# zhangyi-3/UCDIR

Measured on AMD Instinct MI355X. Metric: restored images/sec at 50-step p_sample_loop, 256x256 SID, higher is better.
Workload: dtype bf16

## Files before the change

### ucdir_amd/csrc/conv_ws.hip.h

```cpp
#pragma once
#include <type_traits>
#include "akgm_ws.hip.h"

#ifndef CW_DEPTH
#define CW_DEPTH 1
#endif

struct CvWs {
    static constexpr int PITCH = AkWs::PITCH, HALO = AkWs::HALO, QSTEP = AkWs::QSTEP;
    static constexpr int OFF_TCS = 2 * HALO;
    static constexpr int OFF_SCAL = OFF_TCS + 9 * 64 * 4;
    static constexpr int LDS = OFF_SCAL + 128;
    static constexpr int A_ELEMS = 2 * 36 * 2 * 32 * 8;
};

__global__ __launch_bounds__(HC_THREADS, 2) void conv_ws_kernel(const GemmP p) {
    extern __shared__ __attribute__((aligned(16))) unsigned char smem[];
    float* const tcs = reinterpret_cast<float*>(smem + CvWs::OFF_TCS);
    float* const scal = reinterpret_cast<float*>(smem + CvWs::OFF_SCAL);
    const int tid = threadIdx.x, lane = tid & 63, l31 = lane & 31, hh = lane >> 5;
    const int wave = __builtin_amdgcn_readfirstlane(tid >> 6);
    const int rw = wave & 1, pw = wave >> 1;
    const int prow = l31 >> 4, pcol = (l31 & 15) ^ (prow << 3);
    int lid;
    {
        const int nblk = gridDim.x, bid = blockIdx.x;
        const int q = nblk >> 3, r = nblk & 7, xcd = bid & 7;
        lid = (xcd < r ? xcd * (q + 1) : r * (q + 1) + (xcd - r) * q) + (bid >> 3);
    }
#ifdef UCDIR_TIMING
    const bool dbg_on = p.dbg && (lid == (int)gridDim.x / 2 + 3) && (lane == 0) && (wave == 1 || wave == 5);
    unsigned long long* const dbgp = p.dbg + (wave == 5 ? 256 : 0);
    int dbg_n = 0;
#define CW_STAMP() do { if (dbg_on && dbg_n < 250) dbgp[dbg_n++] = __builtin_amdgcn_s_memtime(); } while (0)
#else
#define CW_STAMP() do {} while (0)
#endif
    CW_STAMP();
    const int tps = p.tiles_x * p.tiles_y;
    const int T = p.nbatch * tps;
    const int t_beg = (int)((long long)lid * T / (int)gridDim.x), t_end = (int)((long long)(lid + 1) * T / (int)gridDim.x);
    if (t_beg >= t_end) return;

    bf16x8_t af[36];
    {
        const bf16_t* Ab = p.A + ((rw * 36 * 2 + hh) * 32 + l31) * 8;
#pragma unroll
        for (int j = 0; j < 36; ++j) af[j] = *reinterpret_cast<const bf16x8_t*>(Ab + j * (2 * 32 * 8));
    }
#pragma unroll
    for (int j = 0; j < 36; ++j) asm volatile("" : "+v"(af[j]));

    int hrel[3], hrel_x = -1;
#pragma unroll
    for (int c3 = 0; c3 < 3; ++c3) {
        const int col = c3 * 8 + (lane >> 3), hp = wave * CvWs::PITCH + col;
        hrel[c3] = col < 18 ? (wave * p.Wp + col) * 64 + (((lane & 7) ^ ((hp >> 1) & 7)) << 3) : -1;
    }
    const int xr = 16 + (wave - 2) / 3, xc3 = (wave - 2) % 3;
    if (wave >= 2) {
        const int col = xc3 * 8 + (lane >> 3), hp = xr * CvWs::PITCH + col;
        hrel_x = col < 18 ? (xr * p.Wp + col) * 64 + (((lane & 7) ^ ((hp >> 1) & 7)) << 3) : -1;
    }
    unsigned ba[3][4];
    {
        const int hp0 = (4 * pw + prow) * CvWs::PITCH + pcol;
#pragma unroll
        for (int kx = 0; kx < 3; ++kx) {
            const int sxh = (((hp0 + kx) >> 1) & 7) ^ hh;
#pragma unroll
            for (int k2 = 0; k2 < 4; ++k2) ba[kx][k2] = ((hp0 + kx) << 7) + (((2 * k2) ^ sxh) << 4);
        }
    }
    const unsigned tc_lane = CvWs::OFF_TCS + (32 * rw + 16 * hh) * 4;
    const unsigned rel_out = (unsigned)(((4 * pw + prow + 1) * p.Wp + pcol + 1) * 64 + 32 * rw + 16 * hh) * 2;

    int b, ty, tx;
    {
        b = t_beg / tps;
        const int r = t_beg - b * tps;
        ty = r / p.tiles_x; tx = r - ty * p.tiles_x;
    }
    auto issue_tile = [&](int nb, int nty, int ntx, int buf) {
        const bf16_t* hb = p.B0 + (long long)nb * p.b0_bstride + (long long)(nty * 16 * p.Wp + ntx * 16) * 64;
        unsigned char* hd = smem + buf * CvWs::HALO;
#pragma unroll
        for (int c3 = 0; c3 < 3; ++c3)
            if (hrel[c3] >= 0) {
                stage16(hb + hrel[c3], hd + (3 * wave + c3) * 1024, lane);
                stage16(hb + (long long)8 * p.Wp * 64 + hrel[c3], hd + (3 * (wave + 8) + c3) * 1024, lane);
            }
        if (wave >= 2) { if (hrel_x >= 0) stage16(hb + hrel_x, hd + (3 * xr + xc3) * 1024, lane); }
    };
    issue_tile(b, ty, tx, 0);

    int b_cur = -1;
    float rstd_a = 1.f;
    stat_t S1 = 0, S2 = 0;
    const int act = p.act;

    f32x16_t acc[2];
    bool pend = false;
    int pb = 0, pty = 0, ptx = 0;
    auto epilogue = [&](int eb, int ety, int etx, const bool wait_dma) {
        const bool interior = ety > 0 && etx > 0 && ety + 1 < p.tiles_y && etx + 1 < p.tiles_x;
        unsigned char* outb = reinterpret_cast<unsigned char*>(reinterpret_cast<bf16_t*>(p.out) + (long long)eb * p.out_bstride + (long long)(ety * 16 * p.Wp + etx * 16) * 64);
        float s1 = 0.f, s2 = 0.f;
        uint4 pk[2][2];
#pragma unroll
        for (int tp = 0; tp < 2; ++tp) {
            unsigned tca = tc_lane + 4 * 256;
            if (!interior) {
                const int r = 4 * pw + 2 * tp + prow, c = pcol;
                const int cy = (ety == 0 && r == 0) ? 0 : ((ety + 1 == p.tiles_y && r == 15) ? 2 : 1);
                const int cx = (etx == 0 && c == 0) ? 0 : ((etx + 1 == p.tiles_x && c == 15) ? 2 : 1);
                tca = tc_lane + (cy * 3 + cx) * 256;
            }
            float v[16];
#pragma unroll
            for (int g4 = 0; g4 < 4; ++g4) {
                const f32x4_t c4 = *reinterpret_cast<const f32x4_t*>(smem + tca + 16 * g4);
#pragma unroll
                for (int e = 0; e < 4; ++e) v[4 * g4 + e] = fmaf(acc[tp][4 * g4 + e], rstd_a, c4[e]);
            }
            if (act == 1) {
#pragma unroll
                for (int i = 0; i < 16; ++i) v[i] = silu_fast(v[i]);
            } else if (act == 2) {
#pragma unroll
                for (int i = 0; i < 16; ++i) v[i] = fmaxf(0.2f * v[i], v[i]);
            }
#pragma unroll
            for (int i = 0; i < 16; ++i) { s1 += v[i]; s2 += v[i] * v[i]; }
            pk[tp][0] = pack8_bf16(v); pk[tp][1] = pack8_bf16(v + 8);
        }
        if (wait_dma) { HC_WAIT(0); }
#pragma unroll
        for (int tp = 0; tp < 2; ++tp) {
            unsigned char* op = outb + rel_out + (long long)tp * (2 * p.Wp * 64 * 2);
            *reinterpret_cast<uint4*>(op) = pk[tp][0];
            *reinterpret_cast<uint4*>(op + 16) = pk[tp][1];
        }
        S1 += stat_fx((double)s1); S2 += stat_fx((double)s2);
    };

    auto tile_loop = [&](auto late_tag) {
    constexpr bool late = decltype(late_tag)::value;
#pragma unroll 1
    for (int t = t_beg; t < t_end; ++t) {
        const int buf = (t - t_beg) & 1;
        const bool last = t + 1 == t_end;
        CW_STAMP();
        if (t == t_beg) { HC_WAIT(0); }
        asm volatile("s_barrier" ::: "memory");
        CW_STAMP();
        if (late && pend) { epilogue(pb, pty, ptx, false); pend = false; }
        if (b != b_cur) {
            if (b_cur >= 0 && p.stats_out) {
                const stat_t a = wave_sum_ll(S1), q2 = wave_sum_ll(S2);
                if (lane == 0) stat_add_fx(p.stats_out, b_cur, a, q2);
            }
            S1 = 0; S2 = 0;
            b_cur = b;
            if (wave == 0) {
                float mean = 0.f, rstd = 1.f;
                if (p.fold) {
                    long long v = 0;
                    if (lane < 2 * UCDIR_STAT_SLOTS) v = p.stats0[(long long)b * (2 * UCDIR_STAT_SLOTS) + lane];
#pragma unroll
                    for (int off = 2; off < 2 * UCDIR_STAT_SLOTS; off <<= 1) v += __shfl_xor(v, off);
                    const long long q = __shfl(v, 1);
                    mean_rstd(stat_val(v), stat_val(q), p.inv_count, mean, rstd);
                }
                if (lane == 0) { scal[0] = mean; scal[1] = rstd; }
            }
            __syncthreads();
            const float mean = scal[0], rstd = scal[1];
            for (int i = tid; i < 9 * 64; i += HC_THREADS) {
                const int cls = i >> 6, f = i & 63;
                float v = p.bias ? p.bias[f] : 0.f;
                if (p.fold) v += p.Tb[(long long)cls * p.tab_ld + f] - mean * rstd * p.Tg[(long long)cls * p.tab_ld + f];
                tcs[i] = v;
            }
            rstd_a = __builtin_bit_cast(float, __builtin_amdgcn_readfirstlane(__builtin_bit_cast(int, p.alpha * (p.fold ? rstd : 1.0f))));
            __syncthreads();
        }
        int nb = b, nty = ty, ntx = tx + 1;
        if (ntx == p.tiles_x) { ntx = 0; if (++nty == p.tiles_y) { nty = 0; ++nb; } }
        CW_STAMP();
        if (!last) issue_tile(nb, nty, ntx, buf ^ 1);
        CW_STAMP();

        if (t != t_beg) {
            const int d = buf ? CvWs::HALO : -CvWs::HALO;
#pragma unroll
            for (int kx = 0; kx < 3; ++kx)
#pragma unroll
                for (int k2 = 0; k2 < 4; ++k2) ba[kx][k2] += d;
        }
#pragma unroll
        for (int tp = 0; tp < 2; ++tp)
#pragma unroll
            for (int e = 0; e < 16; ++e) acc[tp][e] = 0.f;
        bf16x8_t bq[3][2];
        auto read_b = [&](auto jc, bf16x8_t (&dst)[2]) {
            constexpr int j = decltype(jc)::value;
            constexpr int tap = j >> 2, c16 = j & 3;
            constexpr int ky = tap / 3, kx = tap - 3 * ky;
            constexpr int k2 = c16 ^ (ky == 1 ? 2 : 0);
            lds_read16_asm<ky * (CvWs::PITCH * 128)>(dst[0], ba[kx][k2]);
            lds_read16_asm<ky * (CvWs::PITCH * 128) + CvWs::QSTEP>(dst[1], ba[kx][k2]);
        };
        __builtin_amdgcn_sched_barrier(0);
        asm volatile("s_waitcnt lgkmcnt(0)" ::: "memory");
        read_b(std::integral_constant<int, 0>{}, bq[0]);
        read_b(std::integral_constant<int, 1>{}, bq[1]);
        __builtin_amdgcn_s_setprio(1);
        static_for<0, 36>([&](auto jc) {
            constexpr int j = decltype(jc)::value;
            if constexpr (j + 2 < 36) read_b(std::integral_constant<int, j + 2>{}, bq[(j + 2) % 3]);
            constexpr int younger = (j + 2 < 36) ? 4 : ((j + 1 < 36) ? 2 : 0);
            lgkm_wait_asm<younger>();
            const f32x16_t zero = {0.f, 0.f, 0.f, 0.f, 0.f, 0.f, 0.f, 0.f, 0.f, 0.f, 0.f, 0.f, 0.f, 0.f, 0.f, 0.f};
            acc[0] = __builtin_amdgcn_mfma_f32_32x32x16_bf16(af[j], bq[j % 3][0], j ? acc[0] : zero, 0, 0, 0);
            acc[1] = __builtin_amdgcn_mfma_f32_32x32x16_bf16(af[j], bq[j % 3][1], j ? acc[1] : zero, 0, 0, 0);
        });
        __builtin_amdgcn_sched_barrier(0);
        __builtin_amdgcn_s_setprio(0);
        CW_STAMP();
        if (late) { HC_WAIT(0); }
        CW_STAMP();
        if (late) { pend = true; pb = b; pty = ty; ptx = tx; } else epilogue(b, ty, tx, true);
        CW_STAMP();
        b = nb; ty = nty; tx = ntx;
    }
    if (late && pend) epilogue(pb, pty, ptx, false);
#ifdef UCDIR_TIMING
    if (dbg_on) dbgp[255] = dbg_n;
#endif
    };
    if (wave >= 4) tile_loop(std::true_type{}); else tile_loop(std::false_type{});
    if (p.stats_out) {
        const stat_t a = wave_sum_ll(S1), q2 = wave_sum_ll(S2);
        if (lane == 0) stat_add_fx(p.stats_out, b_cur, a, q2);
    }
}
```

### ucdir_amd/csrc/conv_ws128.hip.h

```cpp
#pragma once
#include <type_traits>
#include "conv_ws.hip.h"

struct CvWs128 {
    static constexpr int PITCH = 24;
    static constexpr int PLANE = 10 * PITCH * 128;
    static constexpr int HALO = 2 * PLANE;
    static constexpr int QSTEP = 2 * PITCH * 128;
    static constexpr int OFF_A2 = 2 * HALO;
    static constexpr int A2_BYTES = 2 * 8 * 2 * 32 * 16;
    static constexpr int OFF_TCS = OFF_A2 + A2_BYTES;
    static constexpr int OFF_B2 = OFF_TCS + 9 * 64 * 4;
    static constexpr int OFF_SCAL = OFF_B2 + 64 * 4;
    static constexpr int LDS = OFF_SCAL + 128;
    static constexpr int THREADS = 256;
    static constexpr int DEPTH = 3;
};

__global__ __launch_bounds__(CvWs128::THREADS, 1) void conv_ws128_kernel(const GemmP p) {
    using L = CvWs128;
    extern __shared__ __attribute__((aligned(16))) unsigned char smem[];
    float* const tcs = reinterpret_cast<float*>(smem + L::OFF_TCS);
    float* const b2s = reinterpret_cast<float*>(smem + L::OFF_B2);
    float* const scal = reinterpret_cast<float*>(smem + L::OFF_SCAL);
    const int tid = threadIdx.x, lane = tid & 63, l31 = lane & 31, hh = lane >> 5;
    const int wave = __builtin_amdgcn_readfirstlane(tid >> 6);
    const int rw = wave & 1, pw = wave >> 1;
    const int prow = l31 >> 4, pcol = (l31 & 15) ^ (prow << 3);
    int lid;
    {
        const int nblk = gridDim.x, bid = blockIdx.x;
        const int q = nblk >> 3, r = nblk & 7, xcd = bid & 7;
        lid = (xcd < r ? xcd * (q + 1) : r * (q + 1) + (xcd - r) * q) + (bid >> 3);
    }
#ifdef UCDIR_TIMING
    const bool dbg_on = p.dbg && (lid == (int)gridDim.x / 2 + 3) && (lane == 0) && (wave == 1);
    int dbg_n = 0;
#define C8_STAMP() do { if (dbg_on && dbg_n < 250) p.dbg[dbg_n++] = __builtin_amdgcn_s_memtime(); } while (0)
#else
#define C8_STAMP() do {} while (0)
#endif
    C8_STAMP();
    const int tps = p.tiles_x * p.tiles_y;
    const int T = p.nbatch * tps;
    const int t_beg = (int)((long long)lid * T / (int)gridDim.x), t_end = (int)((long long)(lid + 1) * T / (int)gridDim.x);
    if (t_beg >= t_end) return;

    bf16x8_t af[72];
    {
        const bf16_t* Ab = p.A + ((rw * 72 * 2 + hh) * 32 + l31) * 8;
#pragma unroll
        for (int j = 0; j < 72; ++j) af[j] = *reinterpret_cast<const bf16x8_t*>(Ab + j * (2 * 32 * 8));
    }
#pragma unroll
    for (int j = 0; j < 72; ++j) asm volatile("" : "+v"(af[j]));
    for (int i = tid; i < L::A2_BYTES / 16; i += L::THREADS)
        reinterpret_cast<uint4*>(smem + L::OFF_A2)[i] = reinterpret_cast<const uint4*>(p.alt_A)[i];
    if (tid < 64) b2s[tid] = p.bias2 ? p.bias2[tid] : 0.f;
    __syncthreads();

    unsigned hrel[3];
#pragma unroll
    for (int c3 = 0; c3 < 3; ++c3) {
        const int col = c3 * 8 + (lane >> 3), hp = wave * L::PITCH + col;
        hrel[c3] = col < 18 ? (unsigned)((wave * p.Wp + col) * 64 + (((lane & 7) ^ ((hp >> 1) & 7)) << 3)) * 2u : 0xffffffffu;
    }
    unsigned ba[3][4];
    {
        const int hp0 = (4 * pw + prow) * L::PITCH + pcol;
#pragma unroll
        for (int kx = 0; kx < 3; ++kx) {
            const int sxh = (((hp0 + kx) >> 1) & 7) ^ hh;
#pragma unroll
            for (int k2 = 0; k2 < 4; ++k2) ba[kx][k2] = ((hp0 + kx) << 7) + (((2 * k2) ^ sxh) << 4);
        }
    }
    const unsigned tc_lane = L::OFF_TCS + (32 * rw + 16 * hh) * 4;
    const unsigned b2_lane = L::OFF_B2 + (32 * rw + 16 * hh) * 4;
    const unsigned a2_lane = L::OFF_A2 + ((rw * 8 * 2 + hh) * 32 + l31) * 16;
    const unsigned rel_out = (unsigned)(((4 * pw + prow + 1) * p.Wp + pcol + 1) * 64 + 32 * rw + 16 * hh) * 2;

    int b, ty, tx;
    {
        b = t_beg / tps;
        const int r = t_beg - b * tps;
        ty = r / p.tiles_x; tx = r - ty * p.tiles_x;
    }
    auto issue_tile = [&](int nb, int nty, int ntx, int buf) {
        const long long pix0 = (long long)nty * 8 * p.Wp + ntx * 16;
        const unsigned char* h0 = reinterpret_cast<const unsigned char*>(p.B0 + (long long)nb * p.b0_bstride + pix0 * 64);
        const unsigned char* h1 = reinterpret_cast<const unsigned char*>(p.B1 + (long long)nb * p.b1_bstride + pix0 * 64);
        unsigned char* hd = smem + buf * L::HALO;
        const long long r4 = (long long)4 * p.Wp * 64 * 2;
#pragma unroll
        for (int c3 = 0; c3 < 3; ++c3)
            if (hrel[c3] != 0xffffffffu) {
#pragma unroll
                for (int k = 0; k < 3; ++k)
                    if (k < 2 || wave < 2) {
                        stage16(reinterpret_cast<const bf16_t*>(h0 + k * r4 + hrel[c3]), hd + (3 * (wave + 4 * k) + c3) * 1024, lane);
                        stage16(reinterpret_cast<const bf16_t*>(h1 + k * r4 + hrel[c3]), hd + L::PLANE + (3 * (wave + 4 * k) + c3) * 1024, lane);
                    }
            }
    };
    issue_tile(b, ty, tx, 0);

    int b_cur = -1;
    float rstd_a = 1.f;
    stat_t S1 = 0, S2 = 0;
    const int act = p.act;

#pragma unroll 1
    for (int t = t_beg; t < t_end; ++t) {
        const int buf = (t - t_beg) & 1;
        const bool last = t + 1 == t_end;
        C8_STAMP();
        if (t == t_beg) { HC_WAIT(0); }
        asm volatile("s_barrier" ::: "memory");
        C8_STAMP();
        if (b != b_cur) {
            if (b_cur >= 0 && p.stats_out) {
                const stat_t a = wave_sum_ll(S1), q2 = wave_sum_ll(S2);
                if (lane == 0) stat_add_fx(p.stats_out, b_cur, a, q2);
            }
            S1 = 0; S2 = 0;
            b_cur = b;
            if (wave == 0) {
                float mean = 0.f, rstd = 1.f;
                if (p.fold) {
                    long long v = 0;
                    if (lane < 2 * UCDIR_STAT_SLOTS) {
                        v = p.stats0[(long long)b * (2 * UCDIR_STAT_SLOTS) + lane];
                        if (p.stats1) v += p.stats1[(long long)b * (2 * UCDIR_STAT_SLOTS) + lane];
                    }
#pragma unroll
                    for (int off = 2; off < 2 * UCDIR_STAT_SLOTS; off <<= 1) v += __shfl_xor(v, off);
                    const long long q = __shfl(v, 1);
                    mean_rstd(stat_val(v), stat_val(q), p.inv_count, mean, rstd);
                }
                if (lane == 0) { scal[0] = mean; scal[1] = rstd; }
            }
            __syncthreads();
            const float mean = scal[0], rstd = scal[1];
            for (int i = tid; i < 9 * 64; i += L::THREADS) {
                const int cls = i >> 6, f = i & 63;
                float v = p.bias ? p.bias[f] : 0.f;
                if (p.fold) v += p.Tb[(long long)cls * p.tab_ld + f] - mean * rstd * p.Tg[(long long)cls * p.tab_ld + f];
                tcs[i] = v;
            }
            rstd_a = __builtin_bit_cast(float, __builtin_amdgcn_readfirstlane(__builtin_bit_cast(int, p.alpha * (p.fold ? rstd : 1.0f))));
            __syncthreads();
        }
        int nb = b, nty = ty, ntx = tx + 1;
        if (ntx == p.tiles_x) { ntx = 0; if (++nty == p.tiles_y) { nty = 0; ++nb; } }
        C8_STAMP();

        if (t != t_beg) {
            const int d = buf ? L::HALO : -L::HALO;
#pragma unroll
            for (int kx = 0; kx < 3; ++kx)
#pragma unroll
                for (int k2 = 0; k2 < 4; ++k2) ba[kx][k2] += d;
        }

        f32x16_t acc[2];
        {
            bf16x8_t bq[L::DEPTH + 1][2];
            const long long npix0 = (long long)nty * 8 * p.Wp + ntx * 16;
            const unsigned char* h0 = reinterpret_cast<const unsigned char*>(p.B0 + (long long)nb * p.b0_bstride + npix0 * 64);
            const unsigned char* h1 = reinterpret_cast<const unsigned char*>(p.B1 + (long long)nb * p.b1_bstride + npix0 * 64);
            unsigned char* const hd = smem + (buf ^ 1) * L::HALO;
            const long long r4 = (long long)4 * p.Wp * 64 * 2;
            __builtin_amdgcn_sched_barrier(0);
            asm volatile("s_waitcnt lgkmcnt(0)" ::: "memory");
            static_for<0, L::DEPTH>([&](auto jc) {
                constexpr int j = decltype(jc)::value;
                constexpr int tap = j >> 3, c16 = j & 7, ky = tap / 3, kx = tap - 3 * ky;
                constexpr int off = (c16 >> 2) * L::PLANE + ky * (L::PITCH * 128);
                lds_read16_asm<off>(bq[j][0], ba[kx][(c16 & 3) ^ (ky == 1 ? 2 : 0)]);
                lds_read16_asm<off + L::QSTEP>(bq[j][1], ba[kx][(c16 & 3) ^ (ky == 1 ? 2 : 0)]);
            });
            static_for<0, 72>([&](auto jc) {
                constexpr int j = decltype(jc)::value;
                if constexpr (j + L::DEPTH < 72) {
                    constexpr int jn = j + L::DEPTH;
                    constexpr int tap = jn >> 3, c16 = jn & 7, ky = tap / 3, kx = tap - 3 * ky;
                    constexpr int off = (c16 >> 2) * L::PLANE + ky * (L::PITCH * 128);
                    lds_read16_asm<off>(bq[jn % (L::DEPTH + 1)][0], ba[kx][(c16 & 3) ^ (ky == 1 ? 2 : 0)]);
                    lds_read16_asm<off + L::QSTEP>(bq[jn % (L::DEPTH + 1)][1], ba[kx][(c16 & 3) ^ (ky == 1 ? 2 : 0)]);
                }
                if constexpr (j % 4 == 1 && j / 4 < 18) {
                    constexpr int e = j / 4, c3 = e / 6, k = (e % 6) >> 1, pl = e & 1;
                    if (!last && (k < 2 || wave < 2) && hrel[c3] != 0xffffffffu)
                        stage16(reinterpret_cast<const bf16_t*>((pl ? h1 : h0) + k * r4 + hrel[c3]),
                                hd + pl * L::PLANE + (3 * (wave + 4 * k) + c3) * 1024, lane);
                }
                constexpr int ahead = (71 - j) < L::DEPTH ? (71 - j) : L::DEPTH;
                lgkm_wait_asm<2 * ahead>();
                const f32x16_t zero = {0.f, 0.f, 0.f, 0.f, 0.f, 0.f, 0.f, 0.f, 0.f, 0.f, 0.f, 0.f, 0.f, 0.f, 0.f, 0.f};
                acc[0] = __builtin_amdgcn_mfma_f32_32x32x16_bf16(af[j], bq[j % (L::DEPTH + 1)][0], j ? acc[0] : zero, 0, 0, 0);
                acc[1] = __builtin_amdgcn_mfma_f32_32x32x16_bf16(af[j], bq[j % (L::DEPTH + 1)][1], j ? acc[1] : zero, 0, 0, 0);
            });
            __builtin_amdgcn_sched_barrier(0);
        }
        C8_STAMP();
        f32x16_t acc2[2];
        {
            const f32x16_t zero = {0.f, 0.f, 0.f, 0.f, 0.f, 0.f, 0.f, 0.f, 0.f, 0.f, 0.f, 0.f, 0.f, 0.f, 0.f, 0.f};
#pragma unroll
            for (int j = 0; j < 8; ++j) {
                const bf16x8_t a2 = *reinterpret_cast<const bf16x8_t*>(smem + a2_lane + j * 1024);
                const unsigned a0 = ba[1][(j & 3) ^ 2] + (j >> 2) * L::PLANE + L::PITCH * 128;
                const bf16x8_t b0 = *reinterpret_cast<const bf16x8_t*>(smem + a0);
                const bf16x8_t b1 = *reinterpret_cast<const bf16x8_t*>(smem + a0 + L::QSTEP);
                acc2[0] = __builtin_amdgcn_mfma_f32_32x32x16_bf16(a2, b0, j ? acc2[0] : zero, 0, 0, 0);
                acc2[1] = __builtin_amdgcn_mfma_f32_32x32x16_bf16(a2, b1, j ? acc2[1] : zero, 0, 0, 0);
            }
        }

        C8_STAMP();
        const bool interior = ty > 0 && tx > 0 && ty + 1 < p.tiles_y && tx + 1 < p.tiles_x;
        const long long tile_el = (long long)(ty * 8 * p.Wp + tx * 16) * 64;
        unsigned char* outb = reinterpret_cast<unsigned char*>(reinterpret_cast<bf16_t*>(p.out) + (long long)b * p.out_bstride + tile_el);
        unsigned char* out2b = reinterpret_cast<unsigned char*>(p.out2 + (long long)b * p.out2_bstride + tile_el);
        float s1 = 0.f, s2 = 0.f;
        uint4 pk[2][2], pk2[2][2];
#pragma unroll
        for (int tp = 0; tp < 2; ++tp) {
            unsigned tca = tc_lane + 4 * 256;
            if (!interior) {
                const int r = 4 * pw + 2 * tp + prow, c = pcol;
                const int cy = (ty == 0 && r == 0) ? 0 : ((ty + 1 == p.tiles_y && r == 7) ? 2 : 1);
                const int cx = (tx == 0 && c == 0) ? 0 : ((tx + 1 == p.tiles_x && c == 15) ? 2 : 1);
                tca = tc_lane + (cy * 3 + cx) * 256;
            }
            float v[16], w[16];
#pragma unroll
            for (int g4 = 0; g4 < 4; ++g4) {
                const f32x4_t c4 = *reinterpret_cast<const f32x4_t*>(smem + tca + 16 * g4);
                const f32x4_t d4 = *reinterpret_cast<const f32x4_t*>(smem + b2_lane + 16 * g4);
#pragma unroll
                for (int e = 0; e < 4; ++e) {
                    v[4 * g4 + e] = fmaf(acc[tp][4 * g4 + e], rstd_a, c4[e]);
                    w[4 * g4 + e] = acc2[tp][4 * g4 + e] + d4[e];
                }
            }
            if (act == 1) {
#pragma unroll
                for (int i = 0; i < 16; ++i) v[i] = silu_fast(v[i]);
            } else if (act == 2) {
#pragma unroll
                for (int i = 0; i < 16; ++i) v[i] = fmaxf(0.2f * v[i], v[i]);
            }
#pragma unroll
            for (int i = 0; i < 16; ++i) { s1 += v[i]; s2 += v[i] * v[i]; }
            pk[tp][0] = pack8_bf16(v); pk[tp][1] = pack8_bf16(v + 8);
            pk2[tp][0] = pack8_bf16(w); pk2[tp][1] = pack8_bf16(w + 8);
        }
        C8_STAMP();
        HC_WAIT(0);
        C8_STAMP();
#pragma unroll
        for (int tp = 0; tp < 2; ++tp) {
            const long long o = rel_out + (long long)tp * (2 * p.Wp * 64 * 2);
            *reinterpret_cast<uint4*>(outb + o) = pk[tp][0];
            *reinterpret_cast<uint4*>(outb + o + 16) = pk[tp][1];
            *reinterpret_cast<uint4*>(out2b + o) = pk2[tp][0];
            *reinterpret_cast<uint4*>(out2b + o + 16) = pk2[tp][1];
        }
        S1 += stat_fx((double)s1); S2 += stat_fx((double)s2);
        b = nb; ty = nty; tx = ntx;
    }
#ifdef UCDIR_TIMING
    if (dbg_on) p.dbg[255] = dbg_n;
#endif
    if (p.stats_out) {
        const stat_t a = wave_sum_ll(S1), q2 = wave_sum_ll(S2);
        if (lane == 0) stat_add_fx(p.stats_out, b_cur, a, q2);
    }
}
```

### ucdir_amd/csrc/flash_attn2.hip.h

```cpp
#pragma once
#include "cgemm.hip.h"
#include "asmops.hip.h"

typedef __attribute__((ext_vector_type(8))) _Float16 f16x8_t;
typedef __attribute__((ext_vector_type(2))) uint32_t u32x2_t;

struct FlashP {
    const bf16_t* qkv; long long qkv_bstride; int ld;
    const bf16_t* vt; long long vt_bstride; int Npad;
    int N, C, W;
    float scale_log2e;
    const float* bias;
    const bf16_t* res; long long res_bstride;
    bf16_t* out; long long out_bstride;
    stat_t* stats_out;
    int nq;
    unsigned long long* dbg;
};

#ifdef UCDIR_TIMING
#define FA_STAMP() do { if (dbg_on && dbg_n < 250) p.dbg[dbg_n++] = __builtin_amdgcn_s_memtime(); } while (0)
#else
#define FA_STAMP() do {} while (0)
#endif

#define FA_BQ 128
#define FA_BK 64
#define FA_THREADS 512

__host__ __device__ constexpr int fa_lds_bytes(int C) { return FA_BK * C * 2 * 2 + FA_BQ * FA_BK * 2 + 2048; }

template <bool HALF> struct FaVec { typedef bf16x8_t T; };
template <> struct FaVec<true> { typedef f16x8_t T; };
__device__ __forceinline__ f32x4_t fa_mfma16(const bf16x8_t& a, const bf16x8_t& b, f32x4_t c) { return __builtin_amdgcn_mfma_f32_16x16x32_bf16(a, b, c, 0, 0, 0); }
__device__ __forceinline__ f32x4_t fa_mfma16(const f16x8_t& a, const f16x8_t& b, f32x4_t c) { return __builtin_amdgcn_mfma_f32_16x16x32_f16(a, b, c, 0, 0, 0); }
__device__ __forceinline__ f32x16_t fa_mfma32(const bf16x8_t& a, const bf16x8_t& b, f32x16_t c) { return __builtin_amdgcn_mfma_f32_32x32x16_bf16(a, b, c, 0, 0, 0); }
__device__ __forceinline__ f32x16_t fa_mfma32(const f16x8_t& a, const f16x8_t& b, f32x16_t c) { return __builtin_amdgcn_mfma_f32_32x32x16_f16(a, b, c, 0, 0, 0); }
template <bool HALF>
__device__ __forceinline__ uint32_t fa_pack2(float lo, float hi) {
    if constexpr (HALF) {
        typedef __attribute__((ext_vector_type(2))) _Float16 h2;
        h2 v; v[0] = (_Float16)lo; v[1] = (_Float16)hi;
        return __builtin_bit_cast(uint32_t, v);
    } else return pack2_bf16(lo, hi);
}

template <int OFF, typename V>
__device__ __forceinline__ void fa2_read16(V& v, unsigned addr) {
    asm volatile("ds_read_b128 %0, %1 offset:%2" : "=v"(v) : "v"(addr), "n"(OFF));
}

template <int NC, bool HALF>
__global__ __launch_bounds__(FA_THREADS, 2) void flash_attn2_kernel(const FlashP p) {
    extern __shared__ __attribute__((aligned(16))) unsigned char smem[];
    constexpr int C = 128 * NC;
    constexpr int KROW = C * 2;
    constexpr int NKS = C / 32;
    unsigned char* Kl = smem;
    unsigned char* Vl = smem + FA_BK * KROW;
    unsigned char* Pl = Vl + C * (FA_BK * 2);
    float* rowsc = reinterpret_cast<float*>(Pl + FA_BQ * FA_BK * 2);
    float* red = rowsc + 256;

    const int tid = threadIdx.x, lane = tid & 63;
    const int wave = __builtin_amdgcn_readfirstlane(tid >> 6);
    int lid;
    {
        const int nblk = gridDim.x, bid = blockIdx.x;
        const int q = nblk >> 3, r = nblk & 7, xcd = bid & 7;
        lid = (xcd < r ? xcd * (q + 1) : r * (q + 1) + (xcd - r) * q) + (bid >> 3);
    }
    const int b = lid / p.nq, qtile = lid - b * p.nq;
    const int q0 = qtile * FA_BQ;
    const int N = p.N;
    const int ntiles = (N + FA_BK - 1) / FA_BK;
    const bf16_t* qkvb = p.qkv + (long long)b * p.qkv_bstride;
    const bf16_t* vtb = p.vt + (long long)b * p.vt_bstride;

    const unsigned char* kglob = reinterpret_cast<const unsigned char*>(qkvb + C);
    const unsigned char* vglob = reinterpret_cast<const unsigned char*>(vtb);
    const unsigned krow_bytes = (unsigned)p.ld * 2, vrow_bytes = (unsigned)p.Npad * 2;
    constexpr int NPIECE = 2 * NC;
    auto issue_K_piece = [&](int t, int i) {
        constexpr int LPR = KROW / 16;
        int ln = lane;
        asm volatile("" : "+v"(ln));
        const int inst = i * 8 + wave;
        if constexpr (LPR == 64) {
            int kg = t * FA_BK + inst; kg = kg < N ? kg : N - 1;
            const unsigned char* rowp = kglob + (size_t)__builtin_amdgcn_readfirstlane(kg) * krow_bytes;
            dma16_sbase(rowp, (unsigned)((ln ^ (inst & 15)) << 4), (unsigned)__builtin_amdgcn_readfirstlane(inst * 1024));
        } else {
            const int e = inst * 64 + ln, r = e / LPR, j = e - r * LPR;
            int kg = t * FA_BK + r; kg = kg < N ? kg : N - 1;
            const unsigned off = (unsigned)kg * krow_bytes + (unsigned)((j ^ (r & 15)) << 4);
            dma16_sbase(kglob, off, (unsigned)__builtin_amdgcn_readfirstlane(inst * 1024));
        }
    };
    auto issue_K = [&](int t) {
#pragma unroll
        for (int i = 0; i < NPIECE; ++i) issue_K_piece(t, i);
    };
    auto issue_V_piece = [&](int t, int i) {
        int ln = lane;
        asm volatile("" : "+v"(ln));
        const unsigned lc = (unsigned)((ln & 7) ^ (ln >> 4) ^ ((wave & 1) << 2));
        const unsigned off = (unsigned)(ln >> 3) * vrow_bytes + lc * 16;
        const int inst = i * 8 + wave;
        const unsigned char* rowp = vglob + (size_t)(inst * 8) * vrow_bytes + (size_t)t * (FA_BK * 2);
        dma16_sbase(rowp, off, (unsigned)__builtin_amdgcn_readfirstlane(FA_BK * KROW + inst * 1024));
    };

#ifdef UCDIR_TIMING
    const bool dbg_on = p.dbg && (lid == (int)gridDim.x / 2) && (lane == 0) && (wave == 5);
    int dbg_n = 0;
#endif
    FA_STAMP();
    issue_K(0);

    const int x = lane & 15, g = lane >> 4;
    typedef typename FaVec<HALF>::T vec_t;
    vec_t qf[NKS];
    {
        int qg = q0 + 16 * wave + x; qg = qg < N ? qg : N - 1;
        const bf16_t* qp = qkvb + (long long)qg * p.ld + 8 * g;
#pragma unroll
        for (int ks = 0; ks < NKS; ++ks) qf[ks] = *reinterpret_cast<const vec_t*>(qp + 32 * ks);
    }

    const int kbase = x * KROW, kxor = (g ^ x) << 4;
    const int h = lane >> 5, l31 = lane & 31;
    const int qh = wave >> 2, dq = wave & 3;
    const int vbase = l31 * 128, vxor = (h ^ ((l31 >> 1) & 7)) << 4;
    const int pwbase = (16 * wave + x) * 128 + (g & 1) * 8, pwxor = ((g >> 1) ^ ((x >> 1) & 7)) << 4;

    f32x16_t oacc[NC][2];
#pragma unroll
    for (int dt = 0; dt < NC; ++dt)
#pragma unroll
        for (int qt = 0; qt < 2; ++qt)
#pragma unroll
            for (int e = 0; e < 16; ++e) oacc[dt][qt][e] = 0.f;
    float m_run = -1.0e30f, l_run = 0.f;
    const float c1 = p.scale_log2e;
    constexpr int DPW = 32 * NC;

    for (int t = 0; t < ntiles; ++t) {
        FA_STAMP();
        asm volatile("s_waitcnt vmcnt(0)" ::: "memory");
        FA_STAMP();
        __syncthreads();
        FA_STAMP();
#ifdef FA2_BLOCK_V
        for (int i = 0; i < NPIECE; ++i) issue_V_piece(t, i);
#endif
        f32x4_t sacc[4];
#pragma unroll
        for (int kt = 0; kt < 4; ++kt) sacc[kt] = (f32x4_t){0.f, 0.f, 0.f, 0.f};
        int kx = kxor;
        asm volatile("" : "+v"(kx));
        const unsigned kb2 = (unsigned)kbase | (unsigned)kx;
        auto ka = [&](int c4) { return kb2 ^ (unsigned)(64 * c4); };
        vec_t kf[4];
        __builtin_amdgcn_sched_barrier(0);
        asm volatile("s_waitcnt lgkmcnt(0)" ::: "memory");
        static_for<0, 4>([&](auto ktc) { constexpr int kt = decltype(ktc)::value; fa2_read16<kt * 16 * KROW>(kf[kt], kb2); });
        __builtin_amdgcn_s_setprio(1);
        static_for<0, NKS>([&](auto ksc) {
            constexpr int ks = decltype(ksc)::value;
            static_for<0, 4>([&](auto ktc) {
                constexpr int kt = decltype(ktc)::value;
                lgkm_wait_asm<(ks + 1 < NKS) ? 3 : 3 - kt>();
                sacc[kt] = fa_mfma16(kf[kt], qf[ks], sacc[kt]);
                if constexpr (ks + 1 < NKS) fa2_read16<((ks + 1) >> 2) * 256 + kt * 16 * KROW>(kf[kt], ka((ks + 1) & 3));
            });
#ifndef FA2_BLOCK_V
            if constexpr (ks < NPIECE) issue_V_piece(t, ks);
#endif
        });
        __builtin_amdgcn_s_setprio(0);
#ifdef UCDIR_TIMING
        asm volatile("" :: "v"(sacc[0][0]), "v"(sacc[3][3]));
#endif
        FA_STAMP();
        if (t == ntiles - 1 && (N & (FA_BK - 1))) {
#pragma unroll
            for (int kt = 0; kt < 4; ++kt)
#pragma unroll
                for (int r = 0; r < 4; ++r)
                    if (t * FA_BK + 16 * kt + 4 * g + r >= N) sacc[kt][r] = -3.0e38f;
        }
        float mx = sacc[0][0];
#pragma unroll
        for (int kt = 0; kt < 4; ++kt)
#pragma unroll
            for (int r = 0; r < 4; ++r) mx = fmaxf(mx, sacc[kt][r]);
        { float u = mx, v = mx; asm volatile("s_nop 1\n\tv_permlane16_swap_b32 %0, %1" : "+v"(u), "+v"(v)); mx = fmaxf(u, v); }
        { float u = mx, v = mx; permlane32_swap(u, v); mx = fmaxf(u, v); }
        const float m_new = fmaxf(m_run, mx);
        const float alpha = __builtin_amdgcn_exp2f((m_run - m_new) * c1);
        const float mc = m_new * c1;
        m_run = m_new;
        float psum = 0.f;
        int pwx = pwxor;
        asm volatile("" : "+v"(pwx));
#pragma unroll
        for (int kt = 0; kt < 4; ++kt) {
            float pv[4];
#pragma unroll
            for (int r = 0; r < 4; ++r) { pv[r] = __builtin_amdgcn_exp2f(sacc[kt][r] * c1 - mc); psum += pv[r]; }
            { u32x2_t pk; pk[0] = fa_pack2<HALF>(pv[0], pv[1]); pk[1] = fa_pack2<HALF>(pv[2], pv[3]); *reinterpret_cast<u32x2_t*>(Pl + pwbase + ((32 * kt) ^ pwx)) = pk; }
        }
        l_run = l_run * alpha + psum;
        if (g == 0) rowsc[16 * wave + x] = alpha;
        FA_STAMP();
        asm volatile("s_waitcnt vmcnt(0)" ::: "memory");
        __syncthreads();
        FA_STAMP();
        const bool more = t + 1 < ntiles;
        const int tnext = more ? t + 1 : t;
#ifdef FA2_BLOCK_K
        if (more) issue_K(t + 1);
#endif
        const float a0 = rowsc[64 * qh + l31], a1 = rowsc[64 * qh + 32 + l31];
        const bool rescale = !__all(a0 == 1.0f && a1 == 1.0f);
        int vx = vxor;
        asm volatile("" : "+v"(vx));
        const unsigned pa = ((unsigned)(FA_BK * KROW + C * (FA_BK * 2)) + (unsigned)vbase + (unsigned)((64 * qh) * 128)) | (unsigned)vx;
        const unsigned va = ((unsigned)(FA_BK * KROW) + (unsigned)vbase + (unsigned)(DPW * dq * 128)) | (unsigned)vx;
        vec_t pf[2][2], vf[NC];
        auto pfrag = [&](auto kc, vec_t (&pd)[2]) {
            constexpr int k16 = decltype(kc)::value;
            fa2_read16<0>(pd[0], pa ^ (unsigned)(32 * k16)); fa2_read16<32 * 128>(pd[1], pa ^ (unsigned)(32 * k16));
        };
        __builtin_amdgcn_sched_barrier(0);
        asm volatile("s_waitcnt lgkmcnt(0)" ::: "memory");
        pfrag(std::integral_constant<int, 0>{}, pf[0]);
        static_for<0, NC>([&](auto dc) { constexpr int dt = decltype(dc)::value; fa2_read16<32 * dt * 128>(vf[dt], va); });
        if (rescale) {
#pragma unroll
            for (int dt = 0; dt < NC; ++dt)
#pragma unroll
                for (int e = 0; e < 16; ++e) { oacc[dt][0][e] *= a0; oacc[dt][1][e] *= a1; }
        }
#ifndef FA2_ABL_NOPRIO
        __builtin_amdgcn_s_setprio(1);
#endif
        static_for<0, 4>([&](auto kc) {
            constexpr int k16 = decltype(kc)::value;
#ifndef FA2_ABL_PVNOREAD
            if constexpr (k16 + 1 < 4) pfrag(std::integral_constant<int, k16 + 1>{}, pf[(k16 + 1) & 1]);
#endif
            static_for<0, NC>([&](auto dc) {
                constexpr int dt = decltype(dc)::value;
#ifndef FA2_ABL_PVNOREAD
                lgkm_wait_asm<(k16 + 1 < 4) ? NC + 1 : NC - 1 - dt>();
#else
                if constexpr (k16 == 0 && dt == 0) lgkm_wait_asm<0>();
#endif
#pragma unroll
                for (int qt = 0; qt < 2; ++qt) oacc[dt][qt] = fa_mfma32(vf[dt], pf[k16 & 1][qt], oacc[dt][qt]);
#ifndef FA2_ABL_PVNOREAD
                if constexpr (k16 + 1 < 4) fa2_read16<32 * dt * 128>(vf[dt], va ^ (unsigned)(32 * (k16 + 1)));
#endif
#ifndef FA2_BLOCK_K
                if constexpr (k16 * NC + dt < NPIECE) issue_K_piece(tnext, k16 * NC + dt);
#endif
            });
        });
        __builtin_amdgcn_s_setprio(0);
    }

    asm volatile("s_waitcnt vmcnt(0)" ::: "memory");
#ifdef UCDIR_TIMING
    asm volatile("" :: "v"(oacc[0][0][0]), "v"(oacc[NC - 1][1][15]));
    FA_STAMP();
    if (dbg_on) p.dbg[255] = dbg_n;
#endif
    l_run += __shfl_xor(l_run, 16);
    l_run += __shfl_xor(l_run, 32);
    __syncthreads();
    if (g == 0) rowsc[128 + 16 * wave + x] = 1.0f / l_run;
    __syncthreads();
    float s1 = 0.f, s2 = 0.f;
#pragma unroll
    for (int qt = 0; qt < 2; ++qt) {
        const int ql = 64 * qh + 32 * qt + l31, qg = q0 + ql;
        const float inv_l = rowsc[128 + ql];
        if (qg < N) {
            const int yy = qg / p.W, xx = qg - yy * p.W;
            const long long pix = ((long long)(yy + 1) * (p.W + 2) + xx + 1) * C;
            const bf16_t* rp = p.res + (long long)b * p.res_bstride + pix;
            bf16_t* op = p.out + (long long)b * p.out_bstride + pix;
#pragma unroll
            for (int dt = 0; dt < NC; ++dt)
#pragma unroll
                for (int rq = 0; rq < 4; ++rq) {
                    const int c = DPW * dq + 32 * dt + 8 * rq + 4 * h;
                    const float4 bs = *reinterpret_cast<const float4*>(p.bias + c);
                    const uint2 rv = *reinterpret_cast<const uint2*>(rp + c);
                    float v[4];
                    v[0] = oacc[dt][qt][4 * rq + 0] * inv_l + bs.x + bf2f((bf16_t)(rv.x & 0xffffu));
                    v[1] = oacc[dt][qt][4 * rq + 1] * inv_l + bs.y + bf2f((bf16_t)(rv.x >> 16));
                    v[2] = oacc[dt][qt][4 * rq + 2] * inv_l + bs.z + bf2f((bf16_t)(rv.y & 0xffffu));
                    v[3] = oacc[dt][qt][4 * rq + 3] * inv_l + bs.w + bf2f((bf16_t)(rv.y >> 16));
#pragma unroll
                    for (int i = 0; i < 4; ++i) { s1 += v[i]; s2 += v[i] * v[i]; }
                    *reinterpret_cast<uint2*>(op + c) = make_uint2(pack2_bf16(v[0], v[1]), pack2_bf16(v[2], v[3]));
                }
        }
    }
    if (p.stats_out) {
#pragma unroll
        for (int off = 32; off > 0; off >>= 1) { s1 += __shfl_xor(s1, off); s2 += __shfl_xor(s2, off); }
        if (lane == 0) { red[wave * 2] = s1; red[wave * 2 + 1] = s2; }
        __syncthreads();
        if (tid == 0) {
            float t1 = 0.f, t2 = 0.f;
            for (int w = 0; w < 8; ++w) { t1 += red[w * 2]; t2 += red[w * 2 + 1]; }
            stat_add(p.stats_out, b, t1, t2);
        }
    }
}
```

Before: 38.13.

## Stage attention epilogue residual loads and output stores through LDS with coalesced rows

The flash attention epilogue now DMAs residual rows into swizzled shared memory before the final reduction barrier, preloads bias into registers, applies the bias/residual update in LDS, then writes full 16-byte coalesced rows back to global memory. The goal is to replace scattered 8-byte per-lane residual loads and output stores with wide, row-contiguous transfers that overlap with the l_run reduction. It adds extra barriers and LDS traffic. The conv kernels only gain ablation macros that skip stores for probing.

```diff
diff --git a/ucdir_amd/csrc/conv_ws.hip.h b/ucdir_amd/csrc/conv_ws.hip.h
--- a/ucdir_amd/csrc/conv_ws.hip.h
+++ b/ucdir_amd/csrc/conv_ws.hip.h
@@ -138,8 +138,14 @@
 #pragma unroll
         for (int tp = 0; tp < 2; ++tp) {
             unsigned char* op = outb + rel_out + (long long)tp * (2 * p.Wp * 64 * 2);
+#ifdef CW_ABL_NOSTORE
+            (void)op;
+#pragma unroll
+            for (int i = 0; i < 2; ++i) asm volatile("" :: "v"(pk[tp][i].x), "v"(pk[tp][i].y), "v"(pk[tp][i].z), "v"(pk[tp][i].w));
+#else
             *reinterpret_cast<uint4*>(op) = pk[tp][0];
             *reinterpret_cast<uint4*>(op + 16) = pk[tp][1];
+#endif
         }
         S1 += stat_fx((double)s1); S2 += stat_fx((double)s2);
     };
diff --git a/ucdir_amd/csrc/conv_ws128.hip.h b/ucdir_amd/csrc/conv_ws128.hip.h
--- a/ucdir_amd/csrc/conv_ws128.hip.h
+++ b/ucdir_amd/csrc/conv_ws128.hip.h
@@ -263,10 +263,16 @@
 #pragma unroll
         for (int tp = 0; tp < 2; ++tp) {
             const long long o = rel_out + (long long)tp * (2 * p.Wp * 64 * 2);
+#ifdef CW128_ABL_NOSTORE
+            (void)outb; (void)out2b; (void)o;
+#pragma unroll
+            for (int i = 0; i < 2; ++i) asm volatile("" :: "v"(pk[tp][i].x), "v"(pk[tp][i].y), "v"(pk[tp][i].z), "v"(pk[tp][i].w), "v"(pk2[tp][i].x), "v"(pk2[tp][i].y), "v"(pk2[tp][i].z), "v"(pk2[tp][i].w));
+#else
             *reinterpret_cast<uint4*>(outb + o) = pk[tp][0];
             *reinterpret_cast<uint4*>(outb + o + 16) = pk[tp][1];
             *reinterpret_cast<uint4*>(out2b + o) = pk2[tp][0];
             *reinterpret_cast<uint4*>(out2b + o + 16) = pk2[tp][1];
+#endif
         }
         S1 += stat_fx((double)s1); S2 += stat_fx((double)s2);
         b = nb; ty = nty; tx = ntx;
diff --git a/ucdir_amd/csrc/flash_attn2.hip.h b/ucdir_amd/csrc/flash_attn2.hip.h
--- a/ucdir_amd/csrc/flash_attn2.hip.h
+++ b/ucdir_amd/csrc/flash_attn2.hip.h
@@ -4,6 +4,7 @@
 
 typedef __attribute__((ext_vector_type(8))) _Float16 f16x8_t;
 typedef __attribute__((ext_vector_type(2))) uint32_t u32x2_t;
+typedef __attribute__((ext_vector_type(4))) uint32_t u32x4_t;
 
 struct FlashP {
     const bf16_t* qkv; long long qkv_bstride; int ld;
@@ -277,10 +278,44 @@
     FA_STAMP();
     if (dbg_on) p.dbg[255] = dbg_n;
 #endif
+    constexpr int LPR = KROW / 16;
+    constexpr int NEP = 4 * NC;
+    const unsigned char* resb = reinterpret_cast<const unsigned char*>(p.res + (long long)b * p.res_bstride);
+    unsigned char* outb = reinterpret_cast<unsigned char*>(p.out + (long long)b * p.out_bstride);
+    unsigned eoff[NEP];
+    {
+        unsigned po[2];
+#pragma unroll
+        for (int hq = 0; hq < 2; ++hq) {
+            int qg = q0 + 64 * hq + lane; qg = qg < N ? qg : N - 1;
+            const int yy = qg / p.W, xx = qg - yy * p.W;
+            po[hq] = (unsigned)((yy + 1) * (p.W + 2) + xx + 1) * (unsigned)KROW;
+        }
+#pragma unroll
+        for (int i = 0; i < NEP; ++i) {
+            const int e = (i * 8 + wave) * 64 + lane, r = e / LPR, j = e - r * LPR;
+            eoff[i] = (unsigned)__shfl((int)po[i >= 2 * NC ? 1 : 0], r & 63) + (unsigned)((j ^ (r & 15)) << 4);
+        }
+    }
+    auto issue_res = [&](int i) {
+#ifndef FA2_ABL_NOEPI
+        dma16_sbase(resb, eoff[i], (unsigned)__builtin_amdgcn_readfirstlane((i * 8 + wave) * 1024));
+#endif
+    };
+#pragma unroll
+    for (int i = 0; i < 2 * NC; ++i) issue_res(i);
     l_run += __shfl_xor(l_run, 16);
     l_run += __shfl_xor(l_run, 32);
     __syncthreads();
+#pragma unroll
+    for (int i = 2 * NC; i < NEP; ++i) issue_res(i);
     if (g == 0) rowsc[128 + 16 * wave + x] = 1.0f / l_run;
+    float4 bsv[NC][4];
+#pragma unroll
+    for (int dt = 0; dt < NC; ++dt)
+#pragma unroll
+        for (int rq = 0; rq < 4; ++rq) bsv[dt][rq] = *reinterpret_cast<const float4*>(p.bias + DPW * dq + 32 * dt + 8 * rq + 4 * h);
+    asm volatile("s_waitcnt vmcnt(0)" ::: "memory");
     __syncthreads();
     float s1 = 0.f, s2 = 0.f;
 #pragma unroll
@@ -288,28 +323,45 @@
         const int ql = 64 * qh + 32 * qt + l31, qg = q0 + ql;
         const float inv_l = rowsc[128 + ql];
         if (qg < N) {
-            const int yy = qg / p.W, xx = qg - yy * p.W;
-            const long long pix = ((long long)(yy + 1) * (p.W + 2) + xx + 1) * C;
-            const bf16_t* rp = p.res + (long long)b * p.res_bstride + pix;
-            bf16_t* op = p.out + (long long)b * p.out_bstride + pix;
+            unsigned char* rowp = smem + ql * KROW + 8 * h;
+            const int sw = ql & 15;
 #pragma unroll
             for (int dt = 0; dt < NC; ++dt)
 #pragma unroll
                 for (int rq = 0; rq < 4; ++rq) {
-                    const int c = DPW * dq + 32 * dt + 8 * rq + 4 * h;
-                    const float4 bs = *reinterpret_cast<const float4*>(p.bias + c);
-                    const uint2 rv = *reinterpret_cast<const uint2*>(rp + c);
+                    const float4 bs = bsv[dt][rq];
+                    u32x2_t* sp = reinterpret_cast<u32x2_t*>(rowp + (((4 * NC * dq + 4 * dt + rq) ^ sw) << 4));
+                    const u32x2_t rv = *sp;
                     float v[4];
-                    v[0] = oacc[dt][qt][4 * rq + 0] * inv_l + bs.x + bf2f((bf16_t)(rv.x & 0xffffu));
-                    v[1] = oacc[dt][qt][4 * rq + 1] * inv_l + bs.y + bf2f((bf16_t)(rv.x >> 16));
-                    v[2] = oacc[dt][qt][4 * rq + 2] * inv_l + bs.z + bf2f((bf16_t)(rv.y & 0xffffu));
-                    v[3] = oacc[dt][qt][4 * rq + 3] * inv_l + bs.w + bf2f((bf16_t)(rv.y >> 16));
+                    v[0] = oacc[dt][qt][4 * rq + 0] * inv_l + bs.x + bf2f((bf16_t)(rv[0] & 0xffffu));
+                    v[1] = oacc[dt][qt][4 * rq + 1] * inv_l + bs.y + bf2f((bf16_t)(rv[0] >> 16));
+                    v[2] = oacc[dt][qt][4 * rq + 2] * inv_l + bs.z + bf2f((bf16_t)(rv[1] & 0xffffu));
+                    v[3] = oacc[dt][qt][4 * rq + 3] * inv_l + bs.w + bf2f((bf16_t)(rv[1] >> 16));
 #pragma unroll
                     for (int i = 0; i < 4; ++i) { s1 += v[i]; s2 += v[i] * v[i]; }
-                    *reinterpret_cast<uint2*>(op + c) = make_uint2(pack2_bf16(v[0], v[1]), pack2_bf16(v[2], v[3]));
+                    u32x2_t pk; pk[0] = pack2_bf16(v[0], v[1]); pk[1] = pack2_bf16(v[2], v[3]);
+                    *sp = pk;
                 }
         }
     }
+    __syncthreads();
+#pragma unroll
+    for (int i = 0; i < NEP; ++i) {
+        const int inst = i * 8 + wave, r = (inst * 64 + lane) / LPR;
+        if (q0 + r < N) {
+            const u32x4_t ln = *reinterpret_cast<const u32x4_t*>(smem + inst * 1024 + lane * 16);
+#ifdef FA2_ABL_NOEPI
+            asm volatile("" :: "v"(ln)); (void)outb;
+#else
+            *reinterpret_cast<u32x4_t*>(outb + eoff[i]) = ln;
+#endif
+        }
+    }
+#ifdef UCDIR_TIMING
+    asm volatile("s_waitcnt vmcnt(0)" ::: "memory");
+    FA_STAMP();
+    if (dbg_on) p.dbg[255] = dbg_n;
+#endif
     if (p.stats_out) {
 #pragma unroll
         for (int off = 32; off > 0; off >>= 1) { s1 += __shfl_xor(s1, off); s2 += __shfl_xor(s2, off); }
```

Measured after the change: 38.31 (median of 2 runs). Within noise of the previous version (+0.5%).
